# wangxiaohit/GNNPN-SC

Hardware: AMD Instinct MI355X
Metric: service-composition problems/sec (ML+2PN inference) (higher is better)
Workload: dtype f32-split3xf16 (f32 operands and results; recurrent W_hh.h products: fp32 operands split exactly into 3 x f16, six f16-matrix-core products per term, f32 accumulate; everything else f32 arithmetic)

## Files before the change

### gnnpn-sc_amd/_lib.py

```python
import ctypes
import os
from ctypes import c_char_p, c_double, c_float, c_int, c_int32, c_int64, c_uint32, c_void_p

import torch

_HERE = os.path.dirname(os.path.abspath(__file__))
LIB_PATH = os.environ.get("GNNPN_LIB") or os.path.join(_HERE, "libgnnpn_hip.so")
ABI_VERSION = 9

ACT_NONE, ACT_RELU, ACT_SIGMOID = 0, 1, 2
E_UNSUP = -2
WOA_OK, WOA_ROWS_MISMATCH, WOA_INDEX_ERROR, WOA_NO_SLOTS = 0, 1, 2, 3

_P = c_void_p
_SIGNATURES = {
    "gnnpn_abi_version": (c_int, []),
    "gnnpn_last_error": (c_char_p, []),
    "gnnpn_linear_f32": (c_int, [_P, c_int64, _P, c_int64, _P, _P, _P, c_int, _P, c_int64, c_int64, c_int, c_int, _P]),
    "gnnpn_embed_concat_f32": (c_int, [_P, _P, c_int, c_int, c_int, _P, c_int64, _P]),
    "gnnpn_csr_aggregate_f32": (c_int, [_P, _P, _P, _P, c_int64, _P, _P, _P, _P, c_int, _P, c_int64, c_int32,
                                        c_int32, _P]),
    "gnnpn_csr_aggregate_blocks_f32": (c_int, [_P, _P, _P, _P, c_int64, _P, _P, _P, _P, c_int, _P, c_int64, c_int32,
                                               c_int32, c_int32, _P, _P]),
    "gnnpn_csr_block_row_order": (c_int, [_P, c_int32, c_int32, _P, _P]),
    "gnnpn_csr_tile_plan_geometry": (c_int, [c_int32, c_int32, _P]),
    "gnnpn_csr_tile_plan_rows": (c_int, [_P, _P, _P, c_int32, c_int32, _P, _P, _P, _P, _P, _P]),
    "gnnpn_csr_tile_plan_fill": (c_int, [_P, _P, c_int32, c_int32, _P, _P, _P, _P, c_int64, _P]),
    "gnnpn_csr_aggregate_tiled_f32": (c_int, [_P, _P, _P, _P, _P, c_int64, _P, _P, _P, _P, c_int, _P, c_int64, c_int32, c_int32,
                                              c_int32, _P]),
    "gnnpn_gcn_norm_f32": (c_int, [_P, _P, _P, _P, _P, c_int32, _P]),
    "gnnpn_segment_mean_f32": (c_int, [_P, _P, c_int64, _P, c_int64, c_int32, c_int32, _P]),
    "gnnpn_gin_layer_f32": (c_int, [_P, _P, _P, c_int64, c_int32, _P, _P, _P, _P, _P, c_int32, _P, _P, _P, _P, c_int32, _P, _P, c_int32,
                                    _P, c_int64, c_int64, _P]),
    "gnnpn_split_weights_bytes": (c_int64, [c_int32, c_int32]),
    "gnnpn_lstm_split_weights_bytes": (c_int64, []),
    "gnnpn_lstm_pack_split_weights_f32": (c_int, [_P, _P, _P]),
    "gnnpn_pack_split_weights_f16": (c_int, [_P, c_int64, c_int32, c_int32, _P, _P, _P]),
    "gnnpn_gin_layer_split": (c_int, [_P, _P, _P, c_int64, c_int32, _P, _P, _P, _P, _P, _P, c_int32, _P, _P, _P, _P, _P, c_int32,
                                      _P, _P, _P, c_int32, _P, c_int64, c_int64, _P]),
    "gnnpn_request_branch_f32": (c_int, [_P, c_int32, _P, c_int32, c_int32, _P, _P, _P, c_int32, c_int32, c_int32, _P, c_int32,
                                         _P, _P, _P, _P]),
    "gnnpn_select_candidates": (c_int, [_P, c_int64, _P, _P, _P, _P, _P, _P, _P, c_int32, c_int32, c_int32, _P]),
    "gnnpn_rank_rows": (c_int, [_P, c_int64, _P, c_int32, c_int32, _P]),
    "gnnpn_precision_at_k": (c_int, [_P, c_int64, _P, c_int64, c_int32, c_int32, _P, c_int32, _P, _P]),
    "gnnpn_lstm_encode_f32": (c_int, [c_int, _P, c_int32, c_int32, c_int32, c_int32, c_int32, _P, _P, c_int64, _P]),
    "gnnpn_lstm_encode_workspace_bytes": (c_int64, []),
    "gnnpn_set_option": (c_int, [c_char_p, c_int]),
    "gnnpn_decode_diag": (c_int, [_P, c_int32, c_int32]),
    "gnnpn_coop_reset_staffing": (c_int, []),
    "gnnpn_last_launch_units": (c_int64, []),
    "gnnpn_lds_footprint_kb": (c_int, [c_int]),
    "gnnpn_coop_staffing_count": (c_int, []),
    "gnnpn_bn_train_forward_f32": (c_int, [_P, c_int64, c_int32, _P, _P, c_float, c_float, c_int, _P, _P, _P, _P, _P, _P]),
    "gnnpn_bn_train_backward_f32": (c_int, [_P, _P, _P, _P, _P, c_int64, c_int32, c_int, _P, _P, _P, _P]),
    "gnnpn_bce_sigmoid_f32": (c_int, [_P, _P, c_int64, _P, _P, _P]),
    "gnnpn_dot_f32": (c_int, [_P, _P, c_int64, _P, _P]),
    "gnnpn_embed_grad_f32": (c_int, [_P, c_int64, _P, c_int64, c_int64, c_int32, c_int32, _P, _P]),
    "gnnpn_pointer_decode_f32": (c_int, [c_int, _P, _P, c_float, c_int, c_int32, c_int32, c_int32, c_int32, c_int32,
                                         _P, _P, c_int64, _P]),
    "gnnpn_pointer_decode_workspace_bytes": (c_int64, [c_int32, c_int32, c_int32]),
    "gnnpn_pointer_decode_replicas_f32": (c_int, [_P, _P, c_float, c_int, c_int32, c_int32, c_int32, ctypes.c_uint64, c_int32, c_int32,
                                                  c_int32, _P, _P, c_int64, _P]),
    "gnnpn_replica_seed": (ctypes.c_uint64, [ctypes.c_uint64, c_int32]),
    "gnnpn_best_of_select_f32": (c_int, [c_int32, c_int32, c_int32, _P, _P, _P, _P, _P, _P, _P, _P, _P, _P, _P, _P, _P, _P]),
    "gnnpn_pointer_decode_attn_f32": (c_int, [_P, _P, _P, c_float, c_int, c_int32, c_int32, c_int32, c_int32, _P]),
# ... 180 lines not shown
```

### gnnpn-sc_amd/build.py

```python
import os
import subprocess
import sys
from concurrent.futures import ThreadPoolExecutor

HERE = os.path.dirname(os.path.abspath(__file__))
ROOT = os.path.dirname(HERE)
CSRC = os.path.join(HERE, "csrc")
LIB = os.path.join(HERE, "libgnnpn_hip.so")
SOURCES = ["api.hip", "dense.hip", "graph.hip", "graph_tiled.hip", "gin_layer.hip", "gin_layer_split.hip", "request_branch.hip", "select.hip", "lstm.hip", "lstm_coop.hip", "decode.hip", "decode_coop.hip", "decode_lean.hip", "train.hip", "train_attn.hip", "train_ml.hip", "decode_glimpse.hip", "woa.hip", "woa_prep.hip", "descend.hip", "services.hip", "split_probe.hip"]
HEADERS = [os.path.join(CSRC, "common.h"), os.path.join(CSRC, "graph_lds.h"), os.path.join(CSRC, "gin_aggregate.h"), os.path.join(CSRC, "recurrent.h"), os.path.join(CSRC, "lstm_shared.h"), os.path.join(CSRC, "decode_shared.h"), os.path.join(CSRC, "coop_common.h"), os.path.join(CSRC, "train_common.h"), os.path.join(CSRC, "woa_eval.h"), os.path.join(CSRC, "round5.h"),
           os.path.join(ROOT, "include", "gnnpn_hip.h")]
FLAGS = ["-O3", "--offload-arch=gfx950", "-ffp-contract=off", "-fPIC", "-std=c++17",
         "-I" + os.path.join(ROOT, "include"), "-I" + CSRC] + os.environ.get("GNNPN_EXTRA_HIPCC_FLAGS", "").split()


def _stale(target, deps):
    if not os.path.exists(target):
        return True
    t = os.path.getmtime(target)
    return any(os.path.getmtime(d) > t for d in deps)


def _compile(src):
    obj = os.path.join(HERE, "build", src.replace(".hip", ".o"))
    path = os.path.join(CSRC, src)
    if _stale(obj, [path] + HEADERS):
        subprocess.run(["hipcc"] + FLAGS + ["-c", path, "-o", obj], check=True)
    return obj


def _check_compiler():
    try:
        out = subprocess.run(["hipcc", "--version"], capture_output=True, text=True, check=True).stdout
# ... 44 lines not shown
```

### gnnpn-sc_amd/csrc/select.hip

```cpp
#include <vector>

#include "common.h"

__device__ __forceinline__ unsigned long long rank_key(float score, uint32_t id) {
    return ((unsigned long long)float_order_key(__fadd_rn(score, 0.0f)) << 32) | (0xffffffffu - id);
}

__global__ __launch_bounds__(256) void select_candidates_kernel(
    const float* __restrict__ scores, int64_t ld_scores, const int32_t* __restrict__ cat_ptr,
    const double* __restrict__ qos, const double* __restrict__ local_bounds, const uint8_t* __restrict__ present,
    const double* __restrict__ global_bounds, float* __restrict__ out_rows, int32_t* __restrict__ out_ids,
    int32_t B, int32_t T, int32_t n_per) {
    const int lane = threadIdx.x & 63;
    const int64_t seg = (int64_t)blockIdx.x * 4 + (threadIdx.x >> 6);
    if (seg >= (int64_t)B * T) return;
    const int b = (int)(seg / T), c = (int)(seg - (int64_t)b * T);
    const int s_begin = cat_ptr[c], s_end = cat_ptr[c + 1];
    const bool pres = present[seg] != 0;
    const double* lb = local_bounds + seg * 4;
    const double lo_c = lb[0], hi_c = lb[1], lo_q = lb[2], hi_q = lb[3];
    const float* srow = scores + (int64_t)b * ld_scores;

    unsigned long long last = ~0ull;
    int my_pick = -1;
    int n_found = 0;
    if (pres) {
        for (int r = 0; r < n_per; ++r) {
            unsigned long long best = 0ull;
            for (int s = s_begin + lane; s < s_end; s += 64) {
// ... 11 lines not shown
    }
    const int src_lane = n_found > 0 ? lane % n_found : 0;
    const int id = __shfl(my_pick, src_lane, 64);
    if (lane < n_per) {
        const int64_t pos = (int64_t)b * T * n_per + (int64_t)c * n_per + lane;
        float4 q, tail = make_float4(0.f, 0.f, 0.f, 0.f);
        if (n_found > 0) {
            const double* qs = qos + (int64_t)id * 4;
            q = make_float4((float)qs[0], (float)qs[1], (float)qs[2], (float)qs[3]);
        } else {
            q = make_float4(0.f, 1.f, 1.f, 1.f);
        }
        if (c == 0) {
            const double* g = global_bounds + (int64_t)b * 4;
            tail = make_float4((float)g[0], (float)g[1], (float)g[2], (float)g[3]);
        }
        float4* dst = reinterpret_cast<float4*>(out_rows + pos * 8);
        dst[0] = q;
        dst[1] = tail;
        out_ids[pos] = n_found > 0 ? id : -1;
    }
}

__device__ __forceinline__ unsigned long long row16_max_u64(unsigned long long v) {
#define GNNPN_MAX_STEP(CTRL)                                                                                       \
    {                                                                                                              \
        const unsigned lo = __builtin_amdgcn_update_dpp(0, (int)(unsigned)v, CTRL, 0xF, 0xF, true);                \
        const unsigned hi = __builtin_amdgcn_update_dpp(0, (int)(unsigned)(v >> 32), CTRL, 0xF, 0xF, true);        \
        const unsigned long long o = ((unsigned long long)hi << 32) | lo;                                          \
        v = o > v ? o : v;                                                                                         \
    }
    GNNPN_MAX_STEP(0x121) GNNPN_MAX_STEP(0x122) GNNPN_MAX_STEP(0x124) GNNPN_MAX_STEP(0x128)
    return v;
}
__device__ __forceinline__ unsigned long long row8_max_u64(unsigned long long v) {
    GNNPN_MAX_STEP(0xB1) GNNPN_MAX_STEP(0x4E) GNNPN_MAX_STEP(0x141)
    return v;
#undef GNNPN_MAX_STEP
}

template <int W>
__global__ __launch_bounds__(256) void select_candidates16_kernel(
    const float* __restrict__ scores, int64_t ld_scores, const int32_t* __restrict__ cat_ptr,
    const double* __restrict__ qos, const double* __restrict__ local_bounds, const uint8_t* __restrict__ present,
    const double* __restrict__ global_bounds, float* __restrict__ out_rows, int32_t* __restrict__ out_ids,
    int32_t B, int32_t T, int32_t n_per) {
    const int lane = threadIdx.x & 63, sub = lane & (W - 1);
    const int64_t seg = ((int64_t)blockIdx.x * 4 + (threadIdx.x >> 6)) * (64 / W) + lane / W;
    if (seg >= (int64_t)B * T) return;
    const int b = (int64_t)B * T <= 0x7fffffffll ? (int)((unsigned)seg / (unsigned)T) : (int)(seg / T);
    const int c = (int)(seg - (int64_t)b * T);
    const int s_begin = cat_ptr[c], s_end = cat_ptr[c + 1];
    const bool pres = present[seg] != 0;
    const double* lb = local_bounds + seg * 4;
    const double lo_c = lb[0], hi_c = lb[1], lo_q = lb[2], hi_q = lb[3];
    const float* srow = scores + (int64_t)b * ld_scores;

    auto group_max = [](unsigned long long v) { return W == 16 ? row16_max_u64(v) : row8_max_u64(v); };
    unsigned long long last = ~0ull;
    int my_pick = -1;
    int n_found = 0;
    const bool small = s_end - s_begin <= W;
// ... 183 lines not shown
```

### gnnpn-sc_amd/csrc/torch_ops.cpp

```cpp
#include <ATen/ATen.h>
#include <c10/core/DeviceGuard.h>
#include <c10/hip/HIPStream.h>
#include <torch/library.h>

#include <string>
#include <vector>

#include "gnnpn_hip.h"

namespace {

using at::Tensor;
using OptTensor = std::optional<Tensor>;

#define GNNPN_ON_DEVICE_OF(t)                          \
    TORCH_CHECK((t).is_cuda(), "gnnpn: expected a CUDA tensor (the hot path has no CPU implementation)"); \
    const c10::DeviceGuard device_guard_((t).device()); \
    void* const stream_ = (void*)c10::hip::getCurrentHIPStream((t).device().index()).stream()
#define cur_stream() stream_

void check_rc(int rc, const char* what) { TORCH_CHECK(rc == GNNPN_OK, what, " failed (", rc, "): ", gnnpn_last_error()); }

template <typename T>
const T* cptr(const Tensor& t, at::ScalarType dt, const char* name) {
// ... 157 lines not shown
    check_rc(gnnpn_gin_layer_split(i32(rowptr, "rowptr"), i32(col, "col"), f32(x, "x"), c_in, (int32_t)c_in, f32(eps, "eps"),
                                   cptr<uint8_t>(w1, at::kByte, "w1"), f32(i1, "i1"), f32(b1, "b1"), f32(a1, "a1"), f32(s1, "s1"), (int32_t)h1,
                                   cptr<uint8_t>(w2, at::kByte, "w2"), f32(i2, "i2"), f32(b2, "b2"), f32(a2, "a2"), f32(s2, "s2"), (int32_t)h2,
                                   cptr<uint8_t>(w3, at::kByte, "w3"), f32(i3, "i3"), f32(b3, "b3"), (int32_t)h3, out_f32(out), out.size(1), n,
                                   cur_stream()), "gnnpn_gin_layer_split");
    return out;
}

std::tuple<Tensor, Tensor> segment_topk_feasible(const Tensor& scores, const Tensor& cat_ptr, const Tensor& qos, const Tensor& local_bounds,
                                                 const Tensor& present, const Tensor& global_bounds, int64_t n_per) {
    GNNPN_ON_DEVICE_OF(scores);
    rows2d(scores, "select.scores");
    const int64_t B = scores.size(0), S = scores.size(1), T = cat_ptr.numel() - 1;
    TORCH_CHECK(qos.sizes() == at::IntArrayRef({S, 4}) && local_bounds.sizes() == at::IntArrayRef({B, T, 4}) &&
                    present.sizes() == at::IntArrayRef({B, T}) && global_bounds.sizes() == at::IntArrayRef({B, 4}),
                "select_candidates: inconsistent shapes");
    Tensor rows = new_f32(scores, {B, T * n_per, 8}), ids = new_i32(scores, {B, T * n_per});
    check_rc(gnnpn_select_candidates(f32(scores, "scores"), S, i32(cat_ptr, "cat_ptr"), cptr<double>(qos, at::kDouble, "qos"),
                                     cptr<double>(local_bounds, at::kDouble, "local_bounds"), cptr<uint8_t>(present, at::kByte, "present"),
                                     cptr<double>(global_bounds, at::kDouble, "global_bounds"), out_f32(rows),
                                     static_cast<int32_t*>(ids.data_ptr()), (int32_t)B, (int32_t)T, (int32_t)n_per, cur_stream()),
             "gnnpn_select_candidates");
    return {rows, ids};
}

Tensor rank_rows(const Tensor& scores) {
    GNNPN_ON_DEVICE_OF(scores);
    rows2d(scores, "rank_rows.scores");
    const int64_t B = scores.size(0), S = scores.size(1);
    Tensor ranking = new_i32(scores, {B, S});
    check_rc(gnnpn_rank_rows(f32(scores, "scores"), S, static_cast<int32_t*>(ranking.data_ptr()), (int32_t)B, (int32_t)S, cur_stream()),
             "gnnpn_rank_rows");
    return ranking;
}

Tensor precision_at_k(const Tensor& ranking, const Tensor& labels, at::IntArrayRef ks) {
    GNNPN_ON_DEVICE_OF(labels);
    const int64_t B = labels.size(0), S = labels.size(1);
    std::vector<int32_t> k32(ks.begin(), ks.end());
    Tensor kt = at::tensor(k32, at::TensorOptions().dtype(at::kInt)).to(labels.device());
    Tensor out = new_f32(labels, {B, (int64_t)ks.size()});
    check_rc(gnnpn_precision_at_k(i32(ranking, "ranking"), ranking.size(1), f32(labels, "labels"), S, (int32_t)B, (int32_t)S, i32(kt, "ks"),
                                  (int32_t)ks.size(), out_f32(out), cur_stream()), "gnnpn_precision_at_k");
    return out;
}

// ... 152 lines not shown
}

}

TORCH_LIBRARY(gnnpn, m) {
    m.def("linear(Tensor a, Tensor weight, Tensor? bias=None, Tensor? scale=None, Tensor? shift=None, int act=0) -> Tensor");
    m.def("embed_concat(Tensor x, Tensor table) -> Tensor");
    m.def("csr_aggregate(Tensor rowptr, Tensor col, Tensor? w, Tensor x, Tensor? self_coef=None, Tensor? bias=None, Tensor? scale=None, "
          "Tensor? shift=None, int act=0) -> Tensor");
    m.def("csr_aggregate_blocks(Tensor rowptr, Tensor col, Tensor? w, Tensor x, Tensor? self_coef, Tensor? bias, Tensor? scale, "
          "Tensor? shift, int act, int block_rows, Tensor? row_order=None) -> Tensor");
    m.def("csr_aggregate_tiled(Tensor header, Tensor order, Tensor selfw, Tensor batches, Tensor x, Tensor? self_coef, Tensor? bias, "
          "Tensor? scale, Tensor? shift, int act, int n_rows, int block_rows) -> Tensor");
    m.def("gcn_norm(Tensor rowptr, Tensor col, Tensor w_raw) -> Tensor");
    m.def("segment_mean(Tensor segptr, Tensor x) -> Tensor");
    m.def("request_branch(Tensor x, Tensor table, Tensor rowptr, Tensor col, Tensor seg_ptr, int max_nodes, Tensor[] layer_tensors, "
          "Tensor lin_w_packed, Tensor lin_b, int hidden) -> Tensor");
    m.def("gin_layer(Tensor rowptr, Tensor col, Tensor x, Tensor eps, Tensor w1, Tensor? b1, Tensor? a1, Tensor? s1, Tensor w2, Tensor? b2, "
          "Tensor? a2, Tensor? s2, Tensor? w3=None, Tensor? b3=None) -> Tensor");
    m.def("gin_layer_split(Tensor rowptr, Tensor col, Tensor x, Tensor eps, Tensor w1, Tensor i1, Tensor? b1, Tensor? a1, Tensor? s1, "
          "Tensor w2, Tensor i2, Tensor? b2, Tensor? a2, Tensor? s2, Tensor? w3=None, Tensor? i3=None, Tensor? b3=None) -> Tensor");
    m.def("segment_topk_feasible(Tensor scores, Tensor cat_ptr, Tensor qos, Tensor local_bounds, Tensor present, Tensor global_bounds, "
          "int n_per) -> (Tensor, Tensor)");
    m.def("rank_rows(Tensor scores) -> Tensor");
    m.def("precision_at_k(Tensor ranking, Tensor labels, int[] ks) -> Tensor");
    m.def("attention_logits(Tensor enc_out, Tensor queries, int step, Tensor idx, float tanh_c, bool use_tanh) -> Tensor");
    m.def("qos_reward(Tensor actions, int level) -> Tensor");
    m.def("lstm_encode(Tensor?[] net_tensors, int n_nets, str precision='f32', int impl=0, int lds_kb=0, bool write_through=False, "
          "Tensor? workspace=None, Tensor? status=None, bool paired_start=False) -> Tensor[]");
    m.def("pointer_decode(Tensor?[] net_tensors, int[] latent_from, Tensor inputs, int n_cat, int n_per, float tanh_c=10.0, "
          "bool use_tanh=True, bool want_queries=False, str precision='f32', int impl=0, int lds_kb=0, bool write_through=False, "
          "Tensor? workspace=None, Tensor? status=None, int[] sample_seeds=[], bool paired_start=False) -> Tensor[]");
}

TORCH_LIBRARY_IMPL(gnnpn, CUDA, m) {
    m.impl("linear", linear);
    m.impl("embed_concat", embed_concat);
    m.impl("csr_aggregate", csr_aggregate);
    m.impl("csr_aggregate_blocks", csr_aggregate_blocks);
    m.impl("csr_aggregate_tiled", csr_aggregate_tiled);
    m.impl("gcn_norm", gcn_norm);
    m.impl("segment_mean", segment_mean);
    m.impl("request_branch", request_branch);
    m.impl("gin_layer", gin_layer);
    m.impl("gin_layer_split", gin_layer_split);
    m.impl("segment_topk_feasible", segment_topk_feasible);
    m.impl("rank_rows", rank_rows);
    m.impl("precision_at_k", precision_at_k);
    m.impl("attention_logits", attention_logits);
    m.impl("qos_reward", qos_reward);
    m.impl("lstm_encode", lstm_encode);
    m.impl("pointer_decode", pointer_decode);
}
```

### gnnpn-sc_amd/pipeline.py

```python
import ctypes
import os
from dataclasses import dataclass

import numpy as np
import torch

from . import _lib, custom_ops, graph, ops
from .modelPN import two_level_best_of, two_level_greedy


@dataclass
class DeviceServices:
    x_service: torch.Tensor
    csr: graph.CSR
    cat_ptr: torch.Tensor
    qos: torch.Tensor
    emb_cache: tuple = None

    @staticmethod
    def from_table(table, device):
        ei = torch.from_numpy(np.ascontiguousarray(table.edge_index))
        ea = torch.from_numpy(np.ascontiguousarray(table.edge_attr))
        csr = graph.gcn_csr(ei, ea, table.n_services).to(device)
        return DeviceServices(torch.from_numpy(table.x_service).to(device), csr,
                              torch.from_numpy(np.ascontiguousarray(table.cat_ptr)).to(device),
                              torch.from_numpy(np.ascontiguousarray(table.qos)).to(device))


@dataclass
class DeviceBatch:
    x: torch.Tensor
    wf_csr: graph.CSR
    seg_ptr: torch.Tensor
    local_bounds: torch.Tensor
    present: torch.Tensor
    global_bounds: torch.Tensor
    max_nodes: int = 0

    @property
    def n_problems(self):
# ... 216 lines not shown
        self._side_streams = {}
        warn_partitioned_device(next(low.parameters()).device, self.precision)

    @torch.no_grad()
    def service_embedding(self, services):
        prep = self.net.prepared(services.x_service.device)
        c = services.emb_cache
        if c is None or c[0] is not prep:
            c = services.emb_cache = (prep, self.net.service_embedding(services.x_service, services.csr))
        return c[1]

    @torch.no_grad()
    def scores(self, services, batch):
        return self.net.scores(batch.x, batch.wf_csr, batch.seg_ptr, services.x_service, services.csr,
                               service_emb=self.service_embedding(services) if self.cache_service_embedding else None,
                               max_nodes=batch.max_nodes, dense_precision="split" if self.precision == "split" else "f32")

    @torch.no_grad()
    def candidates(self, services, batch, scores):
        return torch.ops.gnnpn.segment_topk_feasible(scores, services.cat_ptr, services.qos, batch.local_bounds,
                                                     batch.present, batch.global_bounds, self.n_per)

    @torch.no_grad()
    def run(self, services, batch, decode_impl=0, lds_kb=0, ws=None, paired_start=False, write_through=False):
        scores = self.scores(services, batch)
        rows, ids = self.candidates(services, batch, scores)
        if isinstance(ws, (tuple, list)):
            B = rows.shape[0]
            half = half_batch_split(B)
            if len(ws) != 2 or not half:
                raise ops.GnnpnError(f"ML2PNPipeline.run: two half-batches need 2 workspaces and more than 16 problems (got {len(ws)}, {B})")
            cur = torch.cuda.current_stream(rows.device)
            side = self._side_streams.get(rows.device)
            if side is None:
                side = self._side_streams[rows.device] = torch.cuda.Stream(rows.device)
            for net in (self.low, self.high):
                net.actor.packed()
                net.actor.check_precision(self.precision)
            n_cat = rows.shape[1] // self.n_per
            for w in ws:
                w.encode()
                w.decode(max(half, B - half), n_cat, self.n_per)
            side.wait_stream(cur)
            with torch.cuda.stream(side):
                out_b = two_level_greedy(self.low, self.high, rows[half:], precision=self.precision, decode_impl=decode_impl,
                                         lds_kb=lds_kb, ws=ws[1], paired_start=True, write_through=write_through)
            out_a = two_level_greedy(self.low, self.high, rows[:half], precision=self.precision, decode_impl=decode_impl,
                                     lds_kb=lds_kb, ws=ws[0], paired_start=True, write_through=write_through)
            cur.wait_stream(side)
            for v in out_b.values():
                v.record_stream(cur)
            out = {k: torch.cat([out_a[k], out_b[k]]) for k in out_a}
        else:
            out = two_level_greedy(self.low, self.high, rows, precision=self.precision, decode_impl=decode_impl,
                                   lds_kb=lds_kb, ws=ws, paired_start=paired_start, write_through=write_through)
        out.update(scores=scores, pn_inputs=rows, candidate_ids=ids)
        return out

    @torch.no_grad()
    def best_of(self, services, batch, samples, seed=None, decode_impl=0, lds_kb=0, ws=None, write_through=False, return_all=False):
        scores = self.scores(services, batch)
        rows, ids = self.candidates(services, batch, scores)
        out = two_level_best_of(self.low, self.high, rows, samples, seed=seed, precision=self.precision, decode_impl=decode_impl,
                                lds_kb=lds_kb, write_through=write_through, ws=ws, return_all=return_all)
        out.update(scores=scores, pn_inputs=rows, candidate_ids=ids)
        return out

    def refine(self, services, batch, out, popSize, MAX_Iter, reduct=0, seeds=None, min_cost=None, patches=()):
        return refine(services, batch, out, popSize, MAX_Iter, reduct=reduct, seeds=seeds, min_cost=min_cost, patches=patches)

    def descend(self, services, batch, out, max_sweeps=16, reduct=0, min_cost=None, patches=()):
        return descend(services, batch, out, max_sweeps=max_sweeps, reduct=reduct, min_cost=min_cost, patches=patches)

    def descend_starts(self, services, batch, starts, max_sweeps=16, reduct=0, min_cost=None, patches=()):
        return descend_starts(services, batch, starts, max_sweeps=max_sweeps, reduct=reduct, min_cost=min_cost, patches=patches)

    def descend_pairs(self, services, batch, out, max_sweeps=16, max_rounds=4, reduct=0, min_cost=None, patches=()):
        return descend_pairs(services, batch, out, max_sweeps=max_sweeps, max_rounds=max_rounds, reduct=reduct, min_cost=min_cost,
                             patches=patches)

    def descend_pairs_windowed(self, services, batch, out, max_sweeps=16, max_rounds=4, max_span=0, reduct=0, min_cost=None, patches=()):
        return descend_pairs_windowed(services, batch, out, max_sweeps=max_sweeps, max_rounds=max_rounds, max_span=max_span, reduct=reduct,
                                      min_cost=min_cost, patches=patches)

    def descend_pairs_shortlist(self, services, batch, out, max_sweeps=16, max_rounds=4, max_span=0, max_rank=0, reduct=0, min_cost=None,
# ... 346 lines not shown
```

### include/gnnpn_hip.h

```cpp
#ifndef GNNPN_HIP_H
#define GNNPN_HIP_H

#include <stdint.h>

#ifdef __cplusplus
extern "C" {
#endif

#define GNNPN_ABI_VERSION 9

#define GNNPN_OK 0
#define GNNPN_E_ARG (-1)
#define GNNPN_E_UNSUP (-2)
#define GNNPN_E_LAUNCH (-3)

#define GNNPN_ACT_NONE 0
#define GNNPN_ACT_RELU 1
#define GNNPN_ACT_SIGMOID 2

int gnnpn_abi_version(void);
const char* gnnpn_last_error(void);

int gnnpn_linear_f32(const float* A, int64_t lda, const float* W, int64_t ldw, const float* bias,
                     const float* scale, const float* shift, int act, float* C, int64_t ldc,
// ... 58 lines not shown
                          const void* w3, const float* inv3, const float* b3, int32_t h3, float* out, int64_t ldo, int64_t n_rows,
                          void* stream);

typedef struct {
    const float* w0_packed;
    const float* b0;
    const float* bn1_scale;
    const float* bn1_shift;
    const float* w3_packed;
    const float* b3;
    const float* bn2_scale;
    const float* bn2_shift;
    const float* eps;
} gnnpn_gin_layer_t;
int gnnpn_request_branch_f32(const float* x, int32_t nfeat, const float* table, int32_t vocab, int32_t emb,
                             const int32_t* rowptr, const int32_t* col, const int32_t* seg_ptr, int32_t n_graphs,
                             int32_t max_nodes, int32_t n_layers, const gnnpn_gin_layer_t* layers, int32_t hidden,
                             const float* lin_w_packed, const float* lin_b, float* out, void* stream);

int gnnpn_select_candidates(const float* scores, int64_t ld_scores, const int32_t* cat_ptr,
                            const double* qos, const double* local_bounds,
                            const uint8_t* present, const double* global_bounds, float* out_rows,
                            int32_t* out_ids, int32_t B, int32_t T, int32_t n_per, void* stream);

int gnnpn_rank_rows(const float* scores, int64_t ld_scores, int32_t* ranking, int32_t B, int32_t S,
                    void* stream);

int gnnpn_precision_at_k(const int32_t* ranking, int64_t ld_rank, const float* labels, int64_t ld_lab,
                         int32_t B, int32_t S, const int32_t* ks, int32_t n_k, float* out, void* stream);

typedef struct {
    const float* pregates;
    const float* inputs;
    const float* w_in;
    const float* b_in;
    const float* whh_packed;
    const float* bhh;
    float* enc_out;
    float* h_n;
    float* c_n;
    const void* whh_split;
} gnnpn_encode_net_t;

#define GNNPN_PREC_F32 0
#define GNNPN_PREC_F16 1
#define GNNPN_PREC_SPLIT 2
// ... 318 lines not shown
```

Measured before the change: 491,200.

## Fuse service scoring GEMM with per-category candidate selection in one kernel

After: 496,500 (median of 6 runs). 1.1% higher.

```diff
diff --git a/gnnpn-sc_amd/_lib.py b/gnnpn-sc_amd/_lib.py
--- a/gnnpn-sc_amd/_lib.py
+++ b/gnnpn-sc_amd/_lib.py
@@ -41,6 +41,7 @@
     "gnnpn_request_branch_f32": (c_int, [_P, c_int32, _P, c_int32, c_int32, _P, _P, _P, c_int32, c_int32, c_int32, _P, c_int32,
                                          _P, _P, _P, _P]),
     "gnnpn_select_candidates": (c_int, [_P, c_int64, _P, _P, _P, _P, _P, _P, _P, c_int32, c_int32, c_int32, _P]),
+    "gnnpn_score_select_f32": (c_int, [_P, c_int64, _P, _P, _P, c_int32, _P, _P, _P, _P, _P, c_int64, _P, _P, c_int32, c_int32, c_int32, _P]),
     "gnnpn_rank_rows": (c_int, [_P, c_int64, _P, c_int32, c_int32, _P]),
     "gnnpn_precision_at_k": (c_int, [_P, c_int64, _P, c_int64, c_int32, c_int32, _P, c_int32, _P, _P]),
     "gnnpn_lstm_encode_f32": (c_int, [c_int, _P, c_int32, c_int32, c_int32, c_int32, c_int32, _P, _P, c_int64, _P]),
diff --git a/gnnpn-sc_amd/build.py b/gnnpn-sc_amd/build.py
--- a/gnnpn-sc_amd/build.py
+++ b/gnnpn-sc_amd/build.py
@@ -7,8 +7,8 @@
 ROOT = os.path.dirname(HERE)
 CSRC = os.path.join(HERE, "csrc")
 LIB = os.path.join(HERE, "libgnnpn_hip.so")
-SOURCES = ["api.hip", "dense.hip", "graph.hip", "graph_tiled.hip", "gin_layer.hip", "gin_layer_split.hip", "request_branch.hip", "select.hip", "lstm.hip", "lstm_coop.hip", "decode.hip", "decode_coop.hip", "decode_lean.hip", "train.hip", "train_attn.hip", "train_ml.hip", "decode_glimpse.hip", "woa.hip", "woa_prep.hip", "descend.hip", "services.hip", "split_probe.hip"]
-HEADERS = [os.path.join(CSRC, "common.h"), os.path.join(CSRC, "graph_lds.h"), os.path.join(CSRC, "gin_aggregate.h"), os.path.join(CSRC, "recurrent.h"), os.path.join(CSRC, "lstm_shared.h"), os.path.join(CSRC, "decode_shared.h"), os.path.join(CSRC, "coop_common.h"), os.path.join(CSRC, "train_common.h"), os.path.join(CSRC, "woa_eval.h"), os.path.join(CSRC, "round5.h"),
+SOURCES = ["api.hip", "dense.hip", "graph.hip", "graph_tiled.hip", "gin_layer.hip", "gin_layer_split.hip", "request_branch.hip", "select.hip", "score_select.hip", "lstm.hip", "lstm_coop.hip", "decode.hip", "decode_coop.hip", "decode_lean.hip", "train.hip", "train_attn.hip", "train_ml.hip", "decode_glimpse.hip", "woa.hip", "woa_prep.hip", "descend.hip", "services.hip", "split_probe.hip"]
+HEADERS = [os.path.join(CSRC, "common.h"), os.path.join(CSRC, "graph_lds.h"), os.path.join(CSRC, "gin_aggregate.h"), os.path.join(CSRC, "recurrent.h"), os.path.join(CSRC, "lstm_shared.h"), os.path.join(CSRC, "decode_shared.h"), os.path.join(CSRC, "coop_common.h"), os.path.join(CSRC, "train_common.h"), os.path.join(CSRC, "woa_eval.h"), os.path.join(CSRC, "round5.h"), os.path.join(CSRC, "select_keys.h"),
            os.path.join(ROOT, "include", "gnnpn_hip.h")]
 FLAGS = ["-O3", "--offload-arch=gfx950", "-ffp-contract=off", "-fPIC", "-std=c++17",
          "-I" + os.path.join(ROOT, "include"), "-I" + CSRC] + os.environ.get("GNNPN_EXTRA_HIPCC_FLAGS", "").split()
diff --git a/gnnpn-sc_amd/csrc/score_select.hip b/gnnpn-sc_amd/csrc/score_select.hip
--- /dev/null
+++ b/gnnpn-sc_amd/csrc/score_select.hip
@@ -0,0 +1,265 @@
+#include "common.h"
+#include "select_keys.h"
+
+typedef float ss_f32x4 __attribute__((ext_vector_type(4)));
+
+namespace {
+constexpr int PT = 16;
+constexpr int NT = 256;
+constexpr int NW = NT / 64, CSLOTS = NT / 256;
+constexpr int HID = 128;
+constexpr int KB = HID / 16;
+constexpr int LDA = HID + 2;
+constexpr int MAX_TILES = GNNPN_SCORE_SELECT_MAX_TILES;
+constexpr int MAX_CATS = GNNPN_SCORE_SELECT_MAX_CHUNK_CATEGORIES;
+constexpr int LDSC = MAX_TILES * 16 + 16;
+constexpr int CAP = GNNPN_SCORE_SELECT_MAX_CATEGORY;
+constexpr int KPL = CAP / 16;
+
+struct ScoreSelectArgs {
+    const float* xr;
+    const float4* emb;
+    const int32_t* cat_ptr;
+    const int32_t* tile_ptr;
+    const int32_t* chunk_info;
+    const double* qos;
+    const double* local_bounds;
+    const uint8_t* present;
+    const double* global_bounds;
+    float* scores;
+    float* out_rows;
+    int32_t* out_ids;
+    int64_t ldx, ld_scores;
+    int32_t B, T, n_per;
+};
+
+template <int NK>
+__device__ __forceinline__ int select_row(const float* srow, const double* q4, const double* lb, bool pres, int s_begin, int n, int sub,
+                                          int n_per, int& my_pick) {
+    const double lo_c = lb[0], hi_c = lb[1], lo_q = lb[2], hi_q = lb[3];
+    double cost[NK], qual[NK];
+    float score[NK];
+#pragma unroll
+    for (int j = 0; j < NK; ++j) {
+        const int sl = min(sub + 16 * j, n - 1);
+        cost[j] = q4[sl * 4 + 2], qual[j] = q4[sl * 4 + 3], score[j] = srow[sl];
+    }
+    unsigned long long key[NK];
+#pragma unroll
+    for (int j = 0; j < NK; ++j) {
+        const bool ok = pres && sub + 16 * j < n && lo_c <= cost[j] && cost[j] <= hi_c && lo_q <= qual[j] && qual[j] <= hi_q;
+        const unsigned long long k = rank_key(score[j], (uint32_t)(s_begin + sub + 16 * j));
+        key[j] = ok ? k : 0ull;
+    }
+    unsigned long long last = ~0ull;
+    int n_found = 0;
+    for (int r = 0; r < n_per; ++r) {
+        unsigned long long best = 0ull;
+#pragma unroll
+        for (int j = 0; j < NK; ++j) {
+            const unsigned long long k = key[j] < last ? key[j] : 0ull;
+            best = k > best ? k : best;
+        }
+        best = row16_max_u64(best);
+        if (best == 0ull) break;
+        if (sub == r) my_pick = (int)(0xffffffffu - (uint32_t)(best & 0xffffffffu));
+        last = best;
+        ++n_found;
+    }
+    return n_found;
+}
+}
+
+__global__ __launch_bounds__(NT) void score_select_kernel(ScoreSelectArgs a) {
+    __shared__ float As[PT * LDA];
+    __shared__ float sc[PT * LDSC];
+    __shared__ double qs4[MAX_TILES * 16 * 4];
+    __shared__ double lbs[MAX_CATS * PT * 4];
+    __shared__ int cat_s[MAX_CATS + 1], cat_t[MAX_CATS + 1];
+    __shared__ int tile_s[MAX_TILES], tile_e[MAX_TILES];
+    __shared__ unsigned char pres_s[MAX_CATS * PT];
+    const int tid = threadIdx.x, lane = tid & 63, wave = tid >> 6;
+    const int b0 = blockIdx.x * PT;
+    const int32_t* info = a.chunk_info + 8 * blockIdx.y;
+    const int c0 = info[0], c1 = info[1], t0 = info[2], nt = info[3], s0 = info[4], s1 = info[5];
+    if (c0 >= c1) return;
+    const int nc = c1 - c0;
+
+    const float4* wv = a.emb + (size_t)t0 * KB * 64 + lane;
+    float4 bnext[KB];
+    if (wave < nt) {
+#pragma unroll
+        for (int kb = 0; kb < KB; ++kb) bnext[kb] = wv[((size_t)wave * KB + kb) * 64];
+    }
+    for (int f = tid; f < PT * (HID / 4); f += NT) {
+        const int r = f >> 5, k4 = f & 31;
+        float4 v = make_float4(0.f, 0.f, 0.f, 0.f);
+        if (b0 + r < a.B) v = *reinterpret_cast<const float4*>(a.xr + (int64_t)(b0 + r) * a.ldx + 4 * k4);
+        float* d = As + r * LDA + 4 * k4;
+        d[0] = v.x, d[1] = v.y, d[2] = v.z, d[3] = v.w;
+    }
+    for (int i = tid; i < 2 * (s1 - s0); i += NT)
+        *reinterpret_cast<double2*>(qs4 + 2 * i) = *reinterpret_cast<const double2*>(a.qos + (int64_t)s0 * 4 + 2 * i);
+    if (tid <= nc) {
+        const int cs = a.cat_ptr[c0 + tid], ct = a.tile_ptr[c0 + tid];
+        cat_s[tid] = cs;
+        cat_t[tid] = ct - t0;
+        if (tid < nc) {
+            const int ce = a.cat_ptr[c0 + tid + 1], te = a.tile_ptr[c0 + tid + 1];
+            for (int t = ct; t < te; ++t) tile_s[t - t0] = cs + 16 * (t - ct), tile_e[t - t0] = ce;
+        }
+    }
+    for (int i = tid; i < nc * PT; i += NT) {
+        const int cl = i >> 4, pp = i & 15;
+        pres_s[i] = b0 + pp < a.B ? a.present[(int64_t)(b0 + pp) * a.T + c0 + cl] : (unsigned char)0;
+    }
+    for (int i = tid; i < nc * PT * 2; i += NT) {
+        const int cl = i >> 5, pp = (i >> 1) & 15, h = i & 1;
+        double2 v = make_double2(0.0, 0.0);
+        if (b0 + pp < a.B) v = *reinterpret_cast<const double2*>(a.local_bounds + ((int64_t)(b0 + pp) * a.T + c0 + cl) * 4 + 2 * h);
+        *reinterpret_cast<double2*>(lbs + (cl * PT + pp) * 4 + 2 * h) = v;
+    }
+    float4 tail0 = make_float4(0.f, 0.f, 0.f, 0.f);
+    if (c0 == 0 && b0 + ((tid >> 4) & 15) < a.B) {
+        const double* g = a.global_bounds + (int64_t)(b0 + ((tid >> 4) & 15)) * 4;
+        tail0 = make_float4((float)g[0], (float)g[1], (float)g[2], (float)g[3]);
+    }
+    __syncthreads();
+
+    const int c16 = lane & 15, kq = lane >> 4;
+    float afrag[KB][4];
+#pragma unroll
+    for (int kb = 0; kb < KB; ++kb)
+#pragma unroll
+        for (int j = 0; j < 4; ++j) afrag[kb][j] = As[c16 * LDA + 16 * kb + 4 * j + kq];
+    for (int tl = wave; tl < nt; tl += NW) {
+        float4 bf[KB];
+#pragma unroll
+        for (int kb = 0; kb < KB; ++kb) bf[kb] = bnext[kb];
+        if (tl + NW < nt) {
+#pragma unroll
+            for (int kb = 0; kb < KB; ++kb) bnext[kb] = wv[((size_t)(tl + NW) * KB + kb) * 64];
+        }
+        ss_f32x4 acc = {0.f, 0.f, 0.f, 0.f};
+#pragma unroll
+        for (int kb = 0; kb < KB; ++kb) {
+            acc = __builtin_amdgcn_mfma_f32_16x16x4f32(afrag[kb][0], bf[kb].x, acc, 0, 0, 0);
+            acc = __builtin_amdgcn_mfma_f32_16x16x4f32(afrag[kb][1], bf[kb].y, acc, 0, 0, 0);
+            acc = __builtin_amdgcn_mfma_f32_16x16x4f32(afrag[kb][2], bf[kb].z, acc, 0, 0, 0);
+            acc = __builtin_amdgcn_mfma_f32_16x16x4f32(afrag[kb][3], bf[kb].w, acc, 0, 0, 0);
+        }
+        const int s = tile_s[tl] + c16;
+        const bool col_ok = s < tile_e[tl];
+#pragma unroll
+        for (int r = 0; r < 4; ++r) {
+            const float v = epilogue_element(acc[r], false, 0.0f, false, 1.0f, 0.0f, GNNPN_ACT_SIGMOID);
+            const int p = 4 * kq + r;
+            sc[p * LDSC + 16 * tl + c16] = v;
+            if (col_ok && b0 + p < a.B) a.scores[(int64_t)(b0 + p) * a.ld_scores + s] = v;
+        }
+    }
+    __syncthreads();
+
+    const int p = (tid >> 4) & 15, sub = tid & 15;
+    const int b = b0 + p;
+    const bool valid = b < a.B;
+    const int n_per = a.n_per, T = a.T;
+    for (int cl = tid >> 8; cl < nc; cl += CSLOTS) {
+        const int c = c0 + cl;
+        const int s_begin = __builtin_amdgcn_readfirstlane(cat_s[cl]);
+        const int n = __builtin_amdgcn_readfirstlane(cat_s[cl + 1]) - s_begin;
+        const int nk = (n + 15) >> 4;
+        const float* srow = sc + p * LDSC + 16 * __builtin_amdgcn_readfirstlane(cat_t[cl]);
+        const double* q4 = qs4 + (s_begin - s0) * 4;
+        const bool pres = pres_s[cl * PT + p] != 0;
+        int my_pick = -1;
+        int n_found = 0;
+        if (n > 0) {
+            const double* lb = lbs + (cl * PT + p) * 4;
+            if (nk <= 1) n_found = select_row<1>(srow, q4, lb, pres, s_begin, n, sub, n_per, my_pick);
+            else if (nk <= 2) n_found = select_row<2>(srow, q4, lb, pres, s_begin, n, sub, n_per, my_pick);
+            else if (nk <= 4) n_found = select_row<4>(srow, q4, lb, pres, s_begin, n, sub, n_per, my_pick);
+            else if (nk <= 8) n_found = select_row<8>(srow, q4, lb, pres, s_begin, n, sub, n_per, my_pick);
+            else n_found = select_row<KPL>(srow, q4, lb, pres, s_begin, n, sub, n_per, my_pick);
+        }
+        const int src_lane = (lane & ~15) + (n_found > 0 ? sub % n_found : 0);
+        const int id = __shfl(my_pick, src_lane, 64);
+        float4 q = make_float4(0.f, 1.f, 1.f, 1.f);
+        if (n_found > 0 && sub < n_per) {
+            const double* qs = qs4 + (id - s0) * 4;
+            q = make_float4((float)qs[0], (float)qs[1], (float)qs[2], (float)qs[3]);
+        }
+        if (valid && sub < n_per) {
+            const int64_t pos = (int64_t)b * T * n_per + (int64_t)c * n_per + sub;
+            float4* dst = reinterpret_cast<float4*>(a.out_rows + pos * 8);
+            dst[0] = q;
+            dst[1] = c == 0 ? tail0 : make_float4(0.f, 0.f, 0.f, 0.f);
+            a.out_ids[pos] = n_found > 0 ? id : -1;
+        }
+    }
+}
+
+extern "C" int gnnpn_score_select_f32(const float* xr, int64_t ldx, const float* emb_packed, const int32_t* plan_host,
+                                      const int32_t* plan_dev, int32_t plan_words, const double* qos, const double* local_bounds,
+                                      const uint8_t* present, const double* global_bounds, float* scores, int64_t ld_scores,
+                                      float* out_rows, int32_t* out_ids, int32_t B, int32_t hidden, int32_t n_per, void* stream) {
+    GNNPN_REQUIRE(B >= 0, "score_select: bad shape");
+    GNNPN_REQUIRE(plan_host && plan_words >= 4, "score_select: null plan");
+    const int32_t T = plan_host[0], n_chunks = plan_host[1], n_tiles = plan_host[2], S = plan_host[3];
+    GNNPN_REQUIRE(T > 0 && n_chunks > 0 && n_tiles > 0 && S > 0 && (int64_t)plan_words == 4 + 2 * ((int64_t)T + 1) + 9 * (int64_t)n_chunks + 1,
+                  "score_select: plan of %d words does not hold T=%d, n_chunks=%d", plan_words, T, n_chunks);
+    if (hidden != HID || n_per < 1 || n_per > 16)
+        GNNPN_FAIL(GNNPN_E_UNSUP, "score_select: built for hidden = %d and n_per in [1,16] (got hidden %d, n_per %d): use linear + select_candidates",
+                   HID, hidden, n_per);
+    const int32_t* cat = plan_host + 4;
+    const int32_t* tile = cat + T + 1;
+    const int32_t* chunk = tile + T + 1;
+    const int32_t* info = chunk + n_chunks + 1;
+    GNNPN_REQUIRE(cat[0] == 0 && cat[T] == S && tile[0] == 0 && tile[T] == n_tiles && chunk[0] == 0 && chunk[n_chunks] == T,
+                  "score_select: the plan's pointers do not span S=%d services, %d tiles, T=%d categories", S, n_tiles, T);
+    for (int32_t c = 0; c < T; ++c) {
+        const int32_t n = cat[c + 1] - cat[c];
+        GNNPN_REQUIRE(n >= 0 && tile[c + 1] - tile[c] == (n + 15) / 16, "score_select: category %d: %d services in %d tiles", c, n, tile[c + 1] - tile[c]);
+        if (n > CAP) GNNPN_FAIL(GNNPN_E_UNSUP, "score_select: category %d has %d services, the kernel holds %d: use linear + select_candidates", c, n, CAP);
+    }
+    for (int32_t k = 0; k < n_chunks; ++k) {
+        GNNPN_REQUIRE(chunk[k] >= 0 && chunk[k] <= chunk[k + 1] && chunk[k + 1] <= T, "score_select: chunk %d is not a run of categories", k);
+        const int32_t c0 = chunk[k], c1 = chunk[k + 1];
+        GNNPN_REQUIRE(tile[c1] - tile[c0] <= MAX_TILES, "score_select: chunk %d has %d tiles, a workgroup holds %d", k, tile[c1] - tile[c0], MAX_TILES);
+        GNNPN_REQUIRE(c1 - c0 <= MAX_CATS, "score_select: chunk %d has %d categories, a workgroup holds %d", k, c1 - c0, MAX_CATS);
+        const int32_t* r = info + 8 * k;
+        GNNPN_REQUIRE(r[0] == c0 && r[1] == c1 && r[2] == tile[c0] && r[3] == tile[c1] - tile[c0] && r[4] == cat[c0] && r[5] == cat[c1],
+                      "score_select: the record of chunk %d does not repeat the plan's pointers", k);
+    }
+    if (B == 0) return GNNPN_OK;
+    GNNPN_REQUIRE(xr && emb_packed && plan_dev && qos && local_bounds && present && global_bounds && scores && out_rows && out_ids,
+                  "score_select: null operand");
+    GNNPN_REQUIRE(ldx >= HID && ldx % 4 == 0 && gnnpn_aligned(xr, 16) && gnnpn_aligned(emb_packed, 16) && gnnpn_aligned(qos, 16),
+                  "score_select: the request embedding, the packed service embedding and qos must be 16-byte aligned (ldx a multiple of 4)");
+    GNNPN_REQUIRE(ld_scores >= S, "score_select: ld_scores %lld < S = %d", (long long)ld_scores, S);
+    GNNPN_REQUIRE(gnnpn_aligned(out_rows, 16), "score_select: out_rows must be 16-byte aligned");
+    const unsigned ptiles = (unsigned)(((int64_t)B + PT - 1) / PT);
+    GNNPN_REQUIRE(n_chunks <= 65535, "score_select: at most 65535 chunks");
+    ScoreSelectArgs a{};
+    a.xr = xr;
+    a.emb = reinterpret_cast<const float4*>(emb_packed);
+    a.cat_ptr = plan_dev + 4;
+    a.tile_ptr = a.cat_ptr + T + 1;
+    a.chunk_info = a.tile_ptr + T + 1 + n_chunks + 1;
+    a.qos = qos;
+    a.local_bounds = local_bounds;
+    a.present = present;
+    a.global_bounds = global_bounds;
+    a.scores = scores;
+    a.out_rows = out_rows;
+    a.out_ids = out_ids;
+    a.ldx = ldx;
+    a.ld_scores = ld_scores;
+    a.B = B;
+    a.T = T;
+    a.n_per = n_per;
+    hipLaunchKernelGGL(score_select_kernel, dim3(ptiles, (unsigned)n_chunks), dim3(NT), gnnpn_front_lds_pad((const void*)score_select_kernel),
+                       (hipStream_t)stream, a);
+    GNNPN_CHECK_LAUNCH("score_select_f32");
+    return GNNPN_OK;
+}
diff --git a/gnnpn-sc_amd/csrc/select.hip b/gnnpn-sc_amd/csrc/select.hip
--- a/gnnpn-sc_amd/csrc/select.hip
+++ b/gnnpn-sc_amd/csrc/select.hip
@@ -1,10 +1,7 @@
 #include <vector>
 
 #include "common.h"
-
-__device__ __forceinline__ unsigned long long rank_key(float score, uint32_t id) {
-    return ((unsigned long long)float_order_key(__fadd_rn(score, 0.0f)) << 32) | (0xffffffffu - id);
-}
+#include "select_keys.h"
 
 __global__ __launch_bounds__(256) void select_candidates_kernel(
     const float* __restrict__ scores, int64_t ld_scores, const int32_t* __restrict__ cat_ptr,
@@ -62,22 +59,6 @@
     }
 }
 
-__device__ __forceinline__ unsigned long long row16_max_u64(unsigned long long v) {
-#define GNNPN_MAX_STEP(CTRL)                                                                                       \
-    {                                                                                                              \
-        const unsigned lo = __builtin_amdgcn_update_dpp(0, (int)(unsigned)v, CTRL, 0xF, 0xF, true);                \
-        const unsigned hi = __builtin_amdgcn_update_dpp(0, (int)(unsigned)(v >> 32), CTRL, 0xF, 0xF, true);        \
-        const unsigned long long o = ((unsigned long long)hi << 32) | lo;                                          \
-        v = o > v ? o : v;                                                                                         \
-    }
-    GNNPN_MAX_STEP(0x121) GNNPN_MAX_STEP(0x122) GNNPN_MAX_STEP(0x124) GNNPN_MAX_STEP(0x128)
-    return v;
-}
-__device__ __forceinline__ unsigned long long row8_max_u64(unsigned long long v) {
-    GNNPN_MAX_STEP(0xB1) GNNPN_MAX_STEP(0x4E) GNNPN_MAX_STEP(0x141)
-    return v;
-#undef GNNPN_MAX_STEP
-}
 
 template <int W>
 __global__ __launch_bounds__(256) void select_candidates16_kernel(
diff --git a/gnnpn-sc_amd/csrc/select_keys.h b/gnnpn-sc_amd/csrc/select_keys.h
--- /dev/null
+++ b/gnnpn-sc_amd/csrc/select_keys.h
@@ -0,0 +1,23 @@
+#pragma once
+#include "common.h"
+
+__device__ __forceinline__ unsigned long long rank_key(float score, uint32_t id) {
+    return ((unsigned long long)float_order_key(__fadd_rn(score, 0.0f)) << 32) | (0xffffffffu - id);
+}
+
+__device__ __forceinline__ unsigned long long row16_max_u64(unsigned long long v) {
+#define GNNPN_MAX_STEP(CTRL)                                                                                       \
+    {                                                                                                              \
+        const unsigned lo = __builtin_amdgcn_update_dpp(0, (int)(unsigned)v, CTRL, 0xF, 0xF, true);                \
+        const unsigned hi = __builtin_amdgcn_update_dpp(0, (int)(unsigned)(v >> 32), CTRL, 0xF, 0xF, true);        \
+        const unsigned long long o = ((unsigned long long)hi << 32) | lo;                                          \
+        v = o > v ? o : v;                                                                                         \
+    }
+    GNNPN_MAX_STEP(0x121) GNNPN_MAX_STEP(0x122) GNNPN_MAX_STEP(0x124) GNNPN_MAX_STEP(0x128)
+    return v;
+}
+__device__ __forceinline__ unsigned long long row8_max_u64(unsigned long long v) {
+    GNNPN_MAX_STEP(0xB1) GNNPN_MAX_STEP(0x4E) GNNPN_MAX_STEP(0x141)
+    return v;
+#undef GNNPN_MAX_STEP
+}
diff --git a/gnnpn-sc_amd/csrc/torch_ops.cpp b/gnnpn-sc_amd/csrc/torch_ops.cpp
--- a/gnnpn-sc_amd/csrc/torch_ops.cpp
+++ b/gnnpn-sc_amd/csrc/torch_ops.cpp
@@ -203,6 +203,31 @@
                                      static_cast<int32_t*>(ids.data_ptr()), (int32_t)B, (int32_t)T, (int32_t)n_per, cur_stream()),
              "gnnpn_select_candidates");
     return {rows, ids};
+}
+
+std::tuple<Tensor, Tensor, Tensor> score_select(const Tensor& xr, const Tensor& emb_packed, const Tensor& plan_host, const Tensor& plan,
+                                                const Tensor& qos, const Tensor& local_bounds, const Tensor& present,
+                                                const Tensor& global_bounds, int64_t n_per) {
+    GNNPN_ON_DEVICE_OF(xr);
+    rows2d(xr, "score_select.xr");
+    TORCH_CHECK(plan_host.is_cpu() && plan_host.scalar_type() == at::kInt && plan_host.is_contiguous() && plan_host.numel() >= 4,
+                "score_select: plan_host must be a contiguous int32 host tensor");
+    TORCH_CHECK(plan.numel() == plan_host.numel(), "score_select: plan and plan_host differ in length");
+    const int32_t* ph = static_cast<const int32_t*>(plan_host.data_ptr());
+    const int64_t B = xr.size(0), T = ph[0], n_tiles = ph[2], S = ph[3];
+    TORCH_CHECK(T > 0 && S > 0 && n_tiles > 0 && n_per >= 1, "score_select: bad plan header");
+    TORCH_CHECK(emb_packed.numel() == n_tiles * 8 * 64 * 4, "score_select: emb_packed has ", emb_packed.numel(), " elements, the plan's ", n_tiles,
+                " tiles need ", n_tiles * 8 * 64 * 4);
+    TORCH_CHECK(qos.sizes() == at::IntArrayRef({S, 4}) && local_bounds.sizes() == at::IntArrayRef({B, T, 4}) &&
+                    present.sizes() == at::IntArrayRef({B, T}) && global_bounds.sizes() == at::IntArrayRef({B, 4}),
+                "score_select: inconsistent shapes");
+    Tensor scores = new_f32(xr, {B, S}), rows = new_f32(xr, {B, T * n_per, 8}), ids = new_i32(xr, {B, T * n_per});
+    check_rc(gnnpn_score_select_f32(f32(xr, "xr"), xr.size(1), f32(emb_packed, "emb_packed"), ph, i32(plan, "plan"), (int32_t)plan_host.numel(),
+                                    cptr<double>(qos, at::kDouble, "qos"), cptr<double>(local_bounds, at::kDouble, "local_bounds"),
+                                    cptr<uint8_t>(present, at::kByte, "present"), cptr<double>(global_bounds, at::kDouble, "global_bounds"),
+                                    out_f32(scores), S, out_f32(rows), static_cast<int32_t*>(ids.data_ptr()), (int32_t)B, (int32_t)xr.size(1),
+                                    (int32_t)n_per, cur_stream()), "gnnpn_score_select_f32");
+    return {scores, rows, ids};
 }
 
 Tensor rank_rows(const Tensor& scores) {
@@ -401,6 +426,8 @@
           "Tensor w2, Tensor i2, Tensor? b2, Tensor? a2, Tensor? s2, Tensor? w3=None, Tensor? i3=None, Tensor? b3=None) -> Tensor");
     m.def("segment_topk_feasible(Tensor scores, Tensor cat_ptr, Tensor qos, Tensor local_bounds, Tensor present, Tensor global_bounds, "
           "int n_per) -> (Tensor, Tensor)");
+    m.def("score_select(Tensor xr, Tensor emb_packed, Tensor plan_host, Tensor plan, Tensor qos, Tensor local_bounds, Tensor present, "
+          "Tensor global_bounds, int n_per) -> (Tensor, Tensor, Tensor)");
     m.def("rank_rows(Tensor scores) -> Tensor");
     m.def("precision_at_k(Tensor ranking, Tensor labels, int[] ks) -> Tensor");
     m.def("attention_logits(Tensor enc_out, Tensor queries, int step, Tensor idx, float tanh_c, bool use_tanh) -> Tensor");
@@ -424,6 +451,7 @@
     m.impl("gin_layer", gin_layer);
     m.impl("gin_layer_split", gin_layer_split);
     m.impl("segment_topk_feasible", segment_topk_feasible);
+    m.impl("score_select", score_select);
     m.impl("rank_rows", rank_rows);
     m.impl("precision_at_k", precision_at_k);
     m.impl("attention_logits", attention_logits);
diff --git a/gnnpn-sc_amd/pipeline.py b/gnnpn-sc_amd/pipeline.py
--- a/gnnpn-sc_amd/pipeline.py
+++ b/gnnpn-sc_amd/pipeline.py
@@ -5,7 +5,7 @@
 import numpy as np
 import torch
 
-from . import _lib, custom_ops, graph, ops
+from . import _lib, custom_ops, graph, ops, score_plan
 from .modelPN import two_level_best_of, two_level_greedy
 
 
@@ -16,6 +16,7 @@
     cat_ptr: torch.Tensor
     qos: torch.Tensor
     emb_cache: tuple = None
+    score_cache: dict = None
 
     @staticmethod
     def from_table(table, device):
@@ -278,9 +279,46 @@
                                                      batch.present, batch.global_bounds, self.n_per)
 
     @torch.no_grad()
+    def score_select_operands(self, services, batch):
+        if score_plan.unfused_front() or not self.cache_service_embedding:
+            return None
+        hidden = self.net.nodeLin.weight.shape[0]
+        c = services.score_cache
+        if c is None:
+            cat = services.cat_ptr.cpu().numpy()
+            c = services.score_cache = {"cat_ptr": cat, "applies": {}, "plans": {}, "emb": None, "packed": None}
+        key = (int(hidden), int(self.n_per))
+        if key not in c["applies"]:
+            c["applies"][key] = score_plan.applies(c["cat_ptr"], *key)
+        if not c["applies"][key]:
+            return None
+        dev = services.qos.device
+        n_cu = torch.cuda.get_device_properties(dev).multi_processor_count
+        n_chunks = min(len(c["cat_ptr"]) - 1, max(1, n_cu // max(1, (batch.n_problems + 15) // 16)))
+        if n_chunks not in c["plans"]:
+            plan = score_plan.plan_chunks(c["cat_ptr"], n_chunks)
+            c["plans"][n_chunks] = None if plan is None else (plan, *plan.tensors(dev))
+        if c["plans"][n_chunks] is None:
+            return None
+        plan, plan_host, plan_dev = c["plans"][n_chunks]
+        emb = self.service_embedding(services)
+        if c["emb"] is not emb:
+            c["emb"], c["packed"] = emb, score_plan.pack_embedding(emb, plan)
+        return c["packed"], plan_host, plan_dev
+
+    @torch.no_grad()
+    def front(self, services, batch):
+        fused = self.score_select_operands(services, batch)
+        if fused is None:
+            scores = self.scores(services, batch)
+            return (scores, *self.candidates(services, batch, scores))
+        xr = self.net.request_embedding(batch.x, batch.wf_csr, batch.seg_ptr, batch.max_nodes,
+                                        "split" if self.precision == "split" else "f32")
+        return torch.ops.gnnpn.score_select(xr, *fused, services.qos, batch.local_bounds, batch.present, batch.global_bounds, self.n_per)
+
+    @torch.no_grad()
     def run(self, services, batch, decode_impl=0, lds_kb=0, ws=None, paired_start=False, write_through=False):
-        scores = self.scores(services, batch)
-        rows, ids = self.candidates(services, batch, scores)
+        scores, rows, ids = self.front(services, batch)
         if isinstance(ws, (tuple, list)):
             B = rows.shape[0]
             half = half_batch_split(B)
@@ -315,8 +353,7 @@
 
     @torch.no_grad()
     def best_of(self, services, batch, samples, seed=None, decode_impl=0, lds_kb=0, ws=None, write_through=False, return_all=False):
-        scores = self.scores(services, batch)
-        rows, ids = self.candidates(services, batch, scores)
+        scores, rows, ids = self.front(services, batch)
         out = two_level_best_of(self.low, self.high, rows, samples, seed=seed, precision=self.precision, decode_impl=decode_impl,
                                 lds_kb=lds_kb, write_through=write_through, ws=ws, return_all=return_all)
         out.update(scores=scores, pn_inputs=rows, candidate_ids=ids)
diff --git a/gnnpn-sc_amd/score_plan.py b/gnnpn-sc_amd/score_plan.py
--- /dev/null
+++ b/gnnpn-sc_amd/score_plan.py
@@ -0,0 +1,94 @@
+import os
+
+import numpy as np
+
+HIDDEN = 128
+MAX_N_PER = 16
+MAX_CATEGORY = 256
+MAX_TILES = 24
+MAX_CHUNK_CATEGORIES = 16
+MIN_MEAN_CATEGORY = 16
+
+
+def unfused_front():
+    return os.environ.get("GNNPN_UNFUSED_FRONT", "0") == "1"
+
+
+def applies(cat_ptr, hidden, n_per):
+    cat = np.asarray(cat_ptr, dtype=np.int64)
+    sizes = np.diff(cat)
+    return bool(int(hidden) == HIDDEN and 1 <= int(n_per) <= MAX_N_PER and len(sizes) > 0 and cat[0] == 0 and (sizes >= 0).all() and
+                cat[-1] >= MIN_MEAN_CATEGORY * len(sizes) and sizes.max() <= MAX_CATEGORY)
+
+
+def chunk_bounds(cat_ptr, n_chunks):
+    cat = np.asarray(cat_ptr, dtype=np.int64)
+    n = int(n_chunks)
+    if n < 1 or len(cat) < 2:
+        raise ValueError("chunk_bounds: at least one chunk and one category")
+    S = int(cat[-1])
+    targets = np.arange(n + 1, dtype=np.float64) * (S / n)
+    hi = np.clip(np.searchsorted(cat, targets, side="left"), 0, len(cat) - 1)
+    lo = np.clip(hi - 1, 0, len(cat) - 1)
+    bounds = np.where(np.abs(cat[lo] - targets) <= np.abs(cat[hi] - targets), lo, hi)
+    bounds[0], bounds[-1] = 0, len(cat) - 1
+    return np.maximum.accumulate(bounds).astype(np.int32)
+
+
+class ScorePlan:
+
+    def __init__(self, cat_ptr, chunk_ptr):
+        cat = np.asarray(cat_ptr, dtype=np.int32)
+        chunk = np.asarray(chunk_ptr, dtype=np.int32)
+        tile = np.concatenate([[0], np.cumsum((np.diff(cat.astype(np.int64)) + 15) // 16)]).astype(np.int32)
+        self.cat_ptr, self.tile_ptr, self.chunk_ptr = cat, tile, chunk
+        self.n_categories, self.n_chunks, self.n_tiles, self.n_services = len(cat) - 1, len(chunk) - 1, int(tile[-1]), int(cat[-1])
+        lo, hi = chunk[:-1], chunk[1:]
+        zero = np.zeros(self.n_chunks, dtype=np.int32)
+        self.chunk_info = np.stack([lo, hi, tile[lo], tile[hi] - tile[lo], cat[lo], cat[hi], zero, zero], 1).astype(np.int32)
+        self.words = np.concatenate([[self.n_categories, self.n_chunks, self.n_tiles, self.n_services], cat, tile, chunk,
+                                     self.chunk_info.reshape(-1)]).astype(np.int32)
+
+    def chunk_tiles(self):
+        return np.diff(self.tile_ptr[self.chunk_ptr].astype(np.int64))
+
+    def chunk_services(self):
+        return np.diff(self.cat_ptr[self.chunk_ptr].astype(np.int64))
+
+    def fits(self):
+        return bool(self.chunk_tiles().max() <= MAX_TILES and np.diff(self.chunk_ptr).max() <= MAX_CHUNK_CATEGORIES and
+                    np.diff(self.cat_ptr.astype(np.int64)).max() <= MAX_CATEGORY)
+
+    def tensors(self, device):
+        import torch
+        host = torch.from_numpy(self.words.copy())
+        return host, host.to(device)
+
+
+def plan_chunks(cat_ptr, n_chunks):
+    cat = np.asarray(cat_ptr, dtype=np.int64)
+    T = len(cat) - 1
+    n = max(1, int(n_chunks))
+    while True:
+        plan = ScorePlan(cat, chunk_bounds(cat, n) if n != T else np.arange(T + 1))
+        if plan.fits():
+            return plan
+        if n == T:
+            return None
+        n = T if n > T else min(T, n + max(1, n // 4))
+
+
+def pack_embedding(emb, plan):
+    import torch
+    S, K = emb.shape
+    if K != HIDDEN or S != plan.n_services:
+        raise ValueError(f"pack_embedding: [{plan.n_services}, {HIDDEN}] expected, got {tuple(emb.shape)}")
+    sizes = np.diff(plan.cat_ptr.astype(np.int64))
+    n_t = (sizes + 15) // 16
+    cat_of_tile = np.repeat(np.arange(len(sizes)), n_t)
+    first = plan.cat_ptr[cat_of_tile].astype(np.int64) + 16 * (np.arange(plan.n_tiles) - plan.tile_ptr[cat_of_tile])
+    rows = first[:, None] + np.arange(16)[None, :]
+    rows = np.where(rows < plan.cat_ptr[cat_of_tile + 1][:, None], rows, S)
+    padded = torch.cat([emb, torch.zeros((1, K), dtype=emb.dtype, device=emb.device)])
+    v = padded[torch.from_numpy(rows.reshape(-1)).to(emb.device)].view(plan.n_tiles, 16, K // 16, 4, 4)
+    return v.permute(0, 2, 4, 1, 3).reshape(plan.n_tiles, K // 16, 64, 4).contiguous()
diff --git a/include/gnnpn_hip.h b/include/gnnpn_hip.h
--- a/include/gnnpn_hip.h
+++ b/include/gnnpn_hip.h
@@ -104,6 +104,14 @@
                             const double* qos, const double* local_bounds,
                             const uint8_t* present, const double* global_bounds, float* out_rows,
                             int32_t* out_ids, int32_t B, int32_t T, int32_t n_per, void* stream);
+
+#define GNNPN_SCORE_SELECT_MAX_CATEGORY 256
+#define GNNPN_SCORE_SELECT_MAX_TILES 24
+#define GNNPN_SCORE_SELECT_MAX_CHUNK_CATEGORIES 16
+int gnnpn_score_select_f32(const float* xr, int64_t ldx, const float* emb_packed, const int32_t* plan_host,
+                           const int32_t* plan_dev, int32_t plan_words, const double* qos, const double* local_bounds,
+                           const uint8_t* present, const double* global_bounds, float* scores, int64_t ld_scores,
+                           float* out_rows, int32_t* out_ids, int32_t B, int32_t hidden, int32_t n_per, void* stream);
 
 int gnnpn_rank_rows(const float* scores, int64_t ld_scores, int32_t* ranking, int32_t B, int32_t S,
                     void* stream);
```
